# sailordiary/m3f.pytorch

Hardware: AMD Instinct MI355X
Metric: clips/sec (300-frame A+V, fwd+bwd) (higher is better)
Workload: dtype f32 (fp32-accurate products, fp32 accumulate: GEMMs as fp16x3 -- two fp16 terms per scaled operand, three MFMAs, error vs fp64 no larger than an fp32 GEMM's; the forward and backward recurrences at H=512 and H=256 as fp16x3 too (h is bounded; the backward producers split their values under a power-o

## Files before the change

### include/m3t_hip.h

```cpp
#ifndef M3T_HIP_H
#define M3T_HIP_H

#include <stddef.h>
#include <stdint.h>

#ifdef __cplusplus
extern "C" {
#endif

#define M3T_EINVAL 10001
#define M3T_MAX_SCANS 8
#define M3T_ESPIN 10002
#define M3T_SCAN_NO_PERSIST 1
#define M3T_SCAN_WHH 8
#define M3T_SCAN_FP32 4
#define M3T_SCAN_FAULT 16
#define M3T_SCAN_WIDE 32
#define M3T_BF16 2
#define M3T_GEMM_BACKGROUND 1
#define M3T_GEMM_BF16 2
#define M3T_GEMM_HIGH 256
#define M3T_GEMM_F16X3 1024
#define M3T_GEMM_BESIDE_SCAN 512
#define M3T_GEMM_EXCLUSIVE 8
// ... 59 lines not shown
typedef struct {
    const float* A; const float* B; float* C; const float* bias;
    const unsigned long long* amax_a; const unsigned long long* amax_b;
    int accumulate;
} m3t_window_problem;
int m3t_sgemm_window_batch(int n, const m3t_window_problem* problems, int transB, int n_seg, int win_len, int win_stride, int win_off,
                           int N, int K, int lda, int ldb, int ldc, int act, int flags, void* stream);

int m3t_absmax(int n, const float* const* x, const size_t* rows, const int* cols, const size_t* ld,
               unsigned long long* const* slots, void* stream);

int m3t_sgemm_plan(int transA, int M, int N, int K, int seg_len, size_t ws_bytes, int flags, int* kernel, int* splits);

int m3t_colsum(const float* X, int M, int N, int ld, float* out, int accumulate,
               float* ws, size_t ws_bytes, void* stream);

int m3t_transpose(const float* src, int R, int C, int lds, float* dst, int ldd, void* stream);

int m3t_relu_bwd(const float* a, float* dy, size_t n, void* stream);

typedef struct {
    const float* xproj;
    const float* w_hh;
    const float* b_hh;
    float* out;
    float* gates;
    float* h_n;
    int H, reverse, ldx, xoff, ldo, ooff;
} m3t_gru_fwd_desc;

// ... 267 lines not shown
```

### m3f.pytorch_amd/csrc/fuse_loss.hip

```cpp
#include "gru_common.h"
#include <cmath>
#include <cstdlib>
#include <mutex>

namespace {

__device__ __forceinline__ void fuse_weights(float sv, float sa, float& hv, float& ha, float& w0, float& w1) {
    hv = 1.f / (1.f + expf(-sv));
    ha = 1.f / (1.f + expf(-sa));
    const float m = fmaxf(hv, ha);
    const float ev = expf(hv - m), ea = expf(ha - m);
    const float inv = 1.f / (ev + ea);
    w0 = ev * inv;
    w1 = ea * inv;
}

__device__ __forceinline__ float mix2(float w0, float v, float w1, float a) { return fmaf(w0, v, w1 * a); }

__global__ __launch_bounds__(256) void att_fuse_fwd_kernel(const float* __restrict__ s_v, const float* __restrict__ s_a,
                                                           const float* __restrict__ x_v, const float* __restrict__ x_a,
                                                           float* __restrict__ f, int rows, int D, int vec) {
    const int lane = threadIdx.x & 63;
    const int row = blockIdx.x * 4 + (threadIdx.x >> 6);
    if (row >= rows) return;
    float hv, ha, w0, w1;
    fuse_weights(s_v[row], s_a[row], hv, ha, w0, w1);
    const size_t base = (size_t)row * D;
    if (vec) {
        const float4* pv = reinterpret_cast<const float4*>(x_v + base);
        const float4* pa = reinterpret_cast<const float4*>(x_a + base);
        float4* pf = reinterpret_cast<float4*>(f + base);
        for (int i = lane; i < (D >> 2); i += 64) {
            const float4 v = pv[i], a = pa[i];
            pf[i] = make_float4(mix2(w0, v.x, w1, a.x), mix2(w0, v.y, w1, a.y), mix2(w0, v.z, w1, a.z), mix2(w0, v.w, w1, a.w));
        }
    } else {
        for (int i = lane; i < D; i += 64) f[base + i] = mix2(w0, x_v[base + i], w1, x_a[base + i]);
    }
}

__global__ __launch_bounds__(256) void att_fuse_bwd_kernel(const float* __restrict__ df, const float* __restrict__ s_v,
                                                           const float* __restrict__ s_a, const float* __restrict__ x_v,
                                                           const float* __restrict__ x_a, float* __restrict__ ds_v,
                                                           float* __restrict__ ds_a, float* __restrict__ dx_v,
                                                           float* __restrict__ dx_a, int rows, int D, int vec) {
    const int lane = threadIdx.x & 63;
    const int row = blockIdx.x * 4 + (threadIdx.x >> 6);
    if (row >= rows) return;
    float hv, ha, w0, w1;
    fuse_weights(s_v[row], s_a[row], hv, ha, w0, w1);
    const size_t base = (size_t)row * D;
    float d0 = 0.f, d1 = 0.f;
    if (vec) {
// ... 445 lines not shown
}

extern "C" int m3t_sgd_step(float* p, const float* g, float* buf, size_t n, float lr, float momentum, float weight_decay,
                            int step, const float* guard, void* stream) {
    if (n == 0) return 0;
    if (!p || !g || !buf || step < 1) return M3T_EINVAL;
    int blocks = (int)((n + 255) / 256);
    if (blocks > 4096) blocks = 4096;
    sgd_kernel<<<blocks, 256, 0, (hipStream_t)stream>>>(p, g, buf, n, lr, momentum, weight_decay, step == 1, guard);
    M3T_LAUNCH_CHECK();
    return 0;
}

extern "C" int m3t_att_fuse_fwd(const float* s_v, const float* s_a, const float* x_v, const float* x_a, float* f,
                                int rows, int D, void* stream) {
    if (rows <= 0 || D <= 0) return 0;
    if (!s_v || !s_a || !x_v || !x_a || !f) return M3T_EINVAL;
    const int vec = (D % 4 == 0) && (((uintptr_t)x_v | (uintptr_t)x_a | (uintptr_t)f) % 16 == 0);
    att_fuse_fwd_kernel<<<cdiv(rows, 4), 256, 0, (hipStream_t)stream>>>(s_v, s_a, x_v, x_a, f, rows, D, vec);
    M3T_LAUNCH_CHECK();
    return 0;
}

extern "C" int m3t_att_fuse_bwd(const float* df, const float* s_v, const float* s_a, const float* x_v, const float* x_a,
                                float* ds_v, float* ds_a, float* dx_v, float* dx_a, int rows, int D, void* stream) {
    if (rows <= 0 || D <= 0) return 0;
    if (!df || !s_v || !s_a || !x_v || !x_a || !ds_v || !ds_a || !dx_v || !dx_a) return M3T_EINVAL;
    const int vec = (D % 4 == 0) &&
                    (((uintptr_t)x_v | (uintptr_t)x_a | (uintptr_t)df | (uintptr_t)dx_v | (uintptr_t)dx_a) % 16 == 0);
    att_fuse_bwd_kernel<<<cdiv(rows, 4), 256, 0, (hipStream_t)stream>>>(df, s_v, s_a, x_v, x_a, ds_v, ds_a, dx_v, dx_a,
                                                                         rows, D, vec);
    M3T_LAUNCH_CHECK();
    return 0;
}
// ... 86 lines not shown
```

### m3f.pytorch_amd/m3t/_lib.py

```python
import ctypes as C
import os

_HERE = os.path.dirname(os.path.abspath(__file__))
LIB_PATH = os.environ.get("M3T_LIB_PATH") or os.path.join(os.path.dirname(_HERE), "lib", "libm3t_hip.so")
CSRC_DIR = os.path.join(os.path.dirname(_HERE), "csrc")

M3T_EINVAL = 10001
M3T_ESPIN = 10002
M3T_SCAN_NO_PERSIST = 1
M3T_BF16 = 2
M3T_GEMM_BESIDE_SCAN = 512
M3T_GEMM_F16X3 = 1024
M3T_GEMM_HIGH = 256
M3T_GEMM_EXCLUSIVE = 8
M3T_CONV_IMAGES = 4096
M3T_SCAN_FP32 = 4
M3T_SCAN_WHH = 8
M3T_SCAN_FAULT = 16
M3T_SCAN_WIDE = 32
M3T_MAX_SCANS = 8

_f = C.c_void_p
_i = C.c_int
_z = C.c_size_t
# ... 37 lines not shown
    "m3t_conv3d_taps": [_f, _f, _f] + [_i] * 17 + [_f, _f, _f, _z, _f, _s],
    "m3t_sgemm_pre": [_i, _i, _i, _f, _i, _f, _i, _f, _i, _f, _i, _i, _f, _f, _s],
    "m3t_f16x3_split": [_f, _z, _i, _z, _f, _z, _f, _s],
    "m3t_f16x3_split_perm": [_f, _z, _i, _i, _z, _z, _z, _f, _f, _s],
    "m3t_f16x3_image_b": [_f, _i, _i, _z, _f, _f, _s],
    "m3t_sgemm_bimg": [_i, _i, _i, _f, _i, _f, _f, _i, _f, _i, _i, _f, _z, _f, _f, _s],
    "m3t_sgemm_ring": [_i, _i, _i, _i, _i, _f, _i, _f, _i, _f, _i, _f, _i, _i, _i, _i, _i, _i, _f, _z, _i, _f, _f, _i, _s],
    "m3t_conv3d_taps_pre": [_f, _f, _f] + [_i] * 16 + [_f, _f, _f, _z, _f, _s],
    "m3t_conv3d_fwd_taps": [_f, _f, _f, _f] + [_i] * 15 + [_f, _f, _f, _z, _f, _s],
    "m3t_conv3d_fwd_taps4": [_f, _f, _f, _f] + [_i] * 14 + [_f, _f, _f, _z, _f, _s],
    "m3t_planes_to_cl4": [_f, _f, _i, _i, C.c_longlong, _s],
    "m3t_conv3d_wgrad_taps": [_f, _f, _f] + [_i] * 16 + [_f, _f, _f, _z, _s],
    "m3t_amax_out": [C.c_void_p],
    "m3t_colsum": [_f, _i, _i, _i, _f, _i, _f, _z, _s],
    "m3t_transpose": [_f, _i, _i, _i, _f, _i, _s],
    "m3t_relu_bwd": [_f, _f, _z, _s],
    "m3t_gru_scan_fwd": [C.POINTER(GruFwdDesc), _i, _i, _i, _f, _z, _i, _s],
    "m3t_gru_scan_bwd": [C.POINTER(GruBwdDesc), _i, _i, _i, _f, _z, _i, _s],
    "m3t_gru_bwd_prepare_floats": [_i],
    "m3t_gru_bwd_prepare": [C.POINTER(C.c_void_p), _i, _i, _i, C.POINTER(C.c_void_p), _s],
    "m3t_gru_persist_count": [],
    "m3t_gru_scan_workgroups": [_i, _i, _i, _i, _i, _i],
    "m3t_gru_poll_error": [],
    "m3t_gru_error_reset": [],
    "m3t_gru_error_defer": [_i],
    "m3t_gru_inject_error": [_s],
    "m3t_gru_persist_owner": [],
    "m3t_gru_scan_arena": [C.c_void_p, _z],
    "m3t_gru_scan_arena_reset": [C.c_void_p],
    "m3t_gru_scan_after": [C.c_void_p],
# ... 142 lines not shown
```

### m3f.pytorch_amd/m3t/ops.py

```python
import ctypes as C
import os
import sys

import torch

from . import _lib
from ._lib import GruFwdDesc, GruBwdDesc, M3T_MAX_SCANS, M3THipError

_WS = {}
_WS_MIN = 64 << 20

PROFILE = []

import weakref

_GRAD_SINKS = {}


def register_grad_sink(param, view, owner=None):
    _GRAD_SINKS[id(param)] = [weakref.ref(param), view, False, id(owner) if owner is not None else None]


def clear_grad_sinks(owner=None):
    if owner is None:
# ... 431 lines not shown
        if drop is not None and drop[0] > 0:
            Cc = dy.shape[-1]
            _lib.check(lib().m3t_mask_pos_drop(_p(s), _p(dy), _p(out), dy.numel() // Cc, Cc, float(drop[0]), int(drop[1]), _stream()),
                       "m3t_mask_pos_drop")
            return out
        _lib.check(lib().m3t_mask_pos(_p(s), _p(dy), _p(mul), _p(out), dy.numel(), _stream()), "m3t_mask_pos")
        return out
    except BaseException:
        _amax_clear()
        raise


class _Linear(torch.autograd.Function):

    @staticmethod
    def forward(ctx, x, w, b, act, unit=False):
        x = _req(x.contiguous(), "x"); _req(w, "weight")
        K = x.shape[-1]
        N = w.shape[0]
        M = x.numel() // K
        y = torch.empty(x.shape[:-1] + (N,), dtype=x.dtype, device=x.device)
        ctx.prec = _PREC[0]
        slots = None
        ctx.w_slot = None
        if (ctx.prec & _lib.M3T_GEMM_F16X3) and M % 128 == 0 and N % 64 == 0 and K % 32 == 0 and w.is_contiguous():
            slots = amax_slots(3, x.device)
            ctx.w_keep = []
            ctx.w_slot = weight_amax(w, ctx.w_keep)
            ctx.x_slot = amax_one(x.device) if unit else slots.data_ptr()
            todo = ([] if unit else [(x, slots.data_ptr())]) + ([] if ctx.w_slot is not None else [(w, slots.data_ptr() + 8)])
            if todo and not measure_amax(todo):
                slots = None
            elif ctx.w_slot is None:
                ctx.w_slot = slots.data_ptr() + 8
        sgemm(0, 1, M, N, K, x, 0, K, w, 0, K, y, 0, N, bias=b, act=act, prec=ctx.prec, exclusive=True,
              amax=(None, None) if slots is None else (ctx.x_slot, ctx.w_slot))
        ctx.save_for_backward(x, w, y if act else None, slots)
        ctx.act, ctx.has_bias = act, b is not None
        ctx.bias_ref = b if (b is not None and id(b) in _GRAD_SINKS) else None
        ctx.weight_ref = w if id(w) in _GRAD_SINKS else None
        return y

    @staticmethod
    def backward(ctx, dy):
        x, w, y, slots = ctx.saved_tensors
        dy = _req(dy.contiguous(), "dy")
        if ctx.act:
            dy = mask_pos(y, dy)
        K, N = x.shape[-1], w.shape[0]
        M = x.numel() // K
        dx = dw = db = None
        a_x = a_w = a_dy = None
        if slots is not None and measure_amax([(dy, slots.data_ptr() + 16)]):
            a_x, a_w, a_dy = ctx.x_slot, ctx.w_slot, slots.data_ptr() + 16
        if ctx.needs_input_grad[0]:
            dx = torch.empty_like(x)
            sgemm(0, 0, M, K, N, dy, 0, N, w, 0, K, dx, 0, K, prec=ctx.prec, exclusive=True, amax=(a_dy, a_w))
        w_sink = _take_sink(ctx.weight_ref) if (ctx.needs_input_grad[1] and ctx.weight_ref is not None) else None
        b_sink = _take_sink(ctx.bias_ref) if (ctx.has_bias and ctx.needs_input_grad[2] and ctx.bias_ref is not None) else None
        if (ctx.needs_input_grad[1] and ctx.weight_ref is not None and w_sink is None) or \
                (ctx.has_bias and ctx.needs_input_grad[2] and ctx.bias_ref is not None and b_sink is None):
            join_wgrad(x.device)
        wg = wgrad_stream(x.device, _LINEAR_RR[0]) if x.is_cuda else None
        off_chain = on_stream(wg) if wg is not None else None
        if off_chain is not None and (w_sink is not None or b_sink is not None):
            wg.wait_stream(cur_stream())
        if ctx.needs_input_grad[1]:
            if w_sink is not None and off_chain is not None:
                with off_chain:
                    sgemm(1, 0, N, K, M, dy, 0, N, x, 0, K, w_sink, 0, K, prec=ctx.prec, amax=(a_dy, a_x))
                    if slots is not None:
                        slots.record_stream(wg)
            else:
                dw = w_sink if w_sink is not None else torch.empty_like(w)
                sgemm(1, 0, N, K, M, dy, 0, N, x, 0, K, dw, 0, K, prec=ctx.prec, exclusive=True, amax=(a_dy, a_x))
                if w_sink is not None:
                    dw = None
        if ctx.has_bias and ctx.needs_input_grad[2]:
            if b_sink is not None and off_chain is not None:
                with off_chain:
                    colsum(dy, 0, M, N, N, b_sink)
            else:
                db = b_sink if b_sink is not None else torch.empty(N, dtype=x.dtype, device=x.device)
                colsum(dy, 0, M, N, N, db)
                if b_sink is not None:
                    db = None
        if off_chain is not None and (w_sink is not None or b_sink is not None):
            dy.record_stream(wg)
            x.record_stream(wg)
            _WGRAD_PENDING[(x.device.type, x.device.index)] = True
            _LINEAR_RR[0] += 1
        return dx, dw, db, None, None


_LINEAR_RR = [0]


_NBT_PENDING = [None, 0]


def count_batch(counter):
    if counter is None:
        return
    if _NBT_PENDING[0] is not None:
        _NBT_PENDING[0].append(counter)
    else:
        counter.add_(1)


class batch_counters:
# ... 61 lines not shown
    @staticmethod
    def backward(ctx, dy):
        (y,) = ctx.saved_tensors
        return mask_pos(y, _req(dy.contiguous(), "dy"), drop=ctx.drop), None, None


def relu_dropout(y, p, seed=None):
    if p <= 0:
        return y
    if seed is None:
        seed = int(torch.empty(1, dtype=torch.int64).random_().item())
    return _ReluDropout.apply(y, float(p), int(seed))


def linear(x, w, b=None, act=0):
    return _Linear.apply(x, w, b, act, _is_unit(x))


SCAN_PER_STEP = [False]
SCAN_FAULT = [False]
RANGE_PROBE = [[] if os.environ.get("M3T_F16X3_PROBE") == "1" else None]


def _probe_range(tag, t2d):
    a = t2d.abs()
    rmax, cmax, gmax = a.amax(1), a.amax(0), a.max()
    big = torch.full((), float("inf"), device=t2d.device)
    lim = gmax * 2.0 ** -17
    sq = t2d.double() ** 2
    tot = sq.sum()
    past_r, past_c = rmax < lim, cmax < lim
# ... 291 lines not shown
        h_ns = [new(2 * L, B, Hs[s]) for s in range(n_stacks)]
        outs = [[new(B, T, 2 * Hs[s]) for s in range(n_stacks)] for _ in range(L)]
        cat_buf = None
        if cat_hi - cat_lo >= 2:
            cat_buf = new(B, T, sum(2 * Hs[s] for s in range(cat_lo, cat_hi)))
            off = 0
            for s in range(cat_lo, cat_hi):
                outs[L - 1][s] = cat_buf[..., off:off + 2 * Hs[s]]
                off += 2 * Hs[s]
        gates = [[new(2, B, T, 4 * Hs[s]) for s in range(n_stacks)] for _ in range(L)]
        xprojs = [[new(B, T, 6 * Hs[s]) for s in range(n_stacks)] for _ in range(L)]
        main = cur_stream()
        prec = _PREC[0]
        groups = _stream_groups(Hs, B)
        fslots = None
        if (prec & _lib.M3T_GEMM_F16X3) and all(h % 4 == 0 for h in Hs):
            fslots = amax_slots(n_stacks * (1 + 2 * L), dev)
            items = [(xs[s], fslots.data_ptr() + 8 * s) for s in range(n_stacks) if not (unit_mask >> s) & 1]
            wslot = {}
            ctx.w_keep = []
            for l in range(L):
                for s in range(n_stacks):
                    for d in (0, 1):
                        a = weight_amax(params[s][(2 * l + d) * 4], ctx.w_keep)
                        if a is None:
                            a = fslots.data_ptr() + 8 * (n_stacks + (l * n_stacks + s) * 2 + d)
                            items.append((params[s][(2 * l + d) * 4], a))
                        wslot[(l, s, d)] = a
            if not measure_amax(items):
                fslots = None
        one = amax_one(dev)

        def fslot_x(l, s):
            return None if fslots is None else (fslots.data_ptr() + 8 * s if (l == 0 and not (unit_mask >> s) & 1) else one)

        def fslot_w(l, s, d):
            return None if fslots is None else wslot[(l, s, d)]

        alone = not _interleaved(groups) and all(kind == "main" for kind, _ in groups)

        def level_fwd(l, idxs, scan, after=None, wide=False, progress=None):
            descs = []
            for s in idxs:
                H = Hs[s]
                inp = xs[s] if l == 0 else outs[l - 1][s]
                I = inp.shape[-1]
                for d in (0, 1):
                    w_ih, w_hh, b_ih, b_hh = params[s][(2 * l + d) * 4:(2 * l + d) * 4 + 4]
# ... 164 lines not shown
                    ctx.wfq_ev.record(wg1)
                ctx.wfq = wfq
        ctx.n_stacks, ctx.L, ctx.Hs, ctx.B, ctx.T, ctx.prec = n_stacks, L, Hs, B, T, prec
        ctx.unit_mask = unit_mask
        ctx.concurrent = concurrent
        ctx.cat = (cat_lo, cat_hi) if cat_buf is not None else (0, 0)
        saved = []
        for l in range(L):
            for s in range(n_stacks):
                saved += [outs[l][s], gates[l][s]]
        ctx.has_fslots = fslots is not None
        ctx.wslot = wslot if fslots is not None else None
        if fslots is not None:
            for st_ in (side_stream(dev),):
                fslots.record_stream(st_)
            saved.append(fslots)
        ctx.save_for_backward(*(list(tensors) + saved))
        result = []
        for s in range(n_stacks):
            if cat_buf is not None and cat_lo <= s < cat_hi:
                result += [cat_buf if s == cat_lo else new(0), h_ns[s]]
            else:
                result += [outs[L - 1][s], h_ns[s]]
        return tuple(result)

    @staticmethod
    def backward(ctx, *grads):
        n_stacks, L, Hs, B, T = ctx.n_stacks, ctx.L, ctx.Hs, ctx.B, ctx.T
        per = 1 + 8 * L
        st = ctx.saved_tensors
# ... 50 lines not shown
        main = cur_stream()
        groups = _stream_groups(Hs, B)
        cur = {s: douts[s] for s in range(n_stacks)}
        prec = ctx.prec
        wfq = ctx.wfq or {}
        if ctx.wfq_ev is not None:
            main.wait_event(ctx.wfq_ev)
        NSL = _CHUNK_WINDOWS + 1
        bslots = amax_slots(2 * L * n_stacks * NSL, dev) if fslots is not None else None
        one = amax_one(dev)

        def bslot(l, s, d, j=-1):
            return None if bslots is None else bslots.data_ptr() + 8 * (((l * n_stacks + s) * 2 + d) * NSL + 1 + j)

        def fslot_x(l, s):
            return None if fslots is None else (fslots.data_ptr() + 8 * s if (l == 0 and not (ctx.unit_mask >> s) & 1) else one)

        def fslot_w(l, s, d):
            return None if fslots is None else ctx.wslot[(l, s, d)]

        def chunk_plan(l, idxs):
            if bslots is None or len({Hs[i] for i in idxs}) != 1 or 2 * len(idxs) > M3T_MAX_SCANS or not any(need_dx[l][s] for s in idxs):
                return None
            H = Hs[idxs[0]]
            if H % 64 != 0 or any(need_dx[l][s] and layer_io(l, s)[0].shape[-1] % 64 != 0 for s in idxs) or not direct_whh:
                return None
            fl = _scan_flags(dev) | prec | _lib.M3T_SCAN_WHH | _lib.M3T_SCAN_WIDE
            if not lib().m3t_gru_scan_progress_ok(2 * len(idxs), H, B, T, fl, 1):
                return None
            tb = _chunk_bounds(B, T, backward=True)
# ... 221 lines not shown
                    for l in range(L - 1, -1, -1):
                        level_scan(l, idxs, progress=chunk_plan(l, idxs) if (kind == "main" and len(groups) == 1) else None)
                        level_gemms(l, idxs)
            for kind, _ in groups:
                if kind == "side":
                    main.wait_stream(side_stream(dev))
        for key_ in list(held):
            release_held(key_, None)
        weights_sunk = all(sunk[s * per + 1 + (2 * l + d) * 4 + j] for s in range(n_stacks) for l in range(L) for d in (0, 1) for j in (0, 1))
        if weights_sunk:
            for l in range(L):
                for s in range(n_stacks):
                    for t in (dgx[l][s], dgh[l][s]) + tuple(layer_io(l, s)[:2]):
                        for w_ in wgs:
                            t.record_stream(w_)
            for t in (bslots, fslots):
                if t is not None:
                    for w_ in wgs:
                        t.record_stream(w_)
            _WGRAD_PENDING[(dev.type, dev.index)] = True
        else:
            for w_ in wgs:
                main.wait_stream(w_)
        for s in range(n_stacks):
            out_grads[s * per] = dinp[0][s]
        return (None, None, None, None, None) + tuple(None if sunk[i] else g for i, g in enumerate(out_grads))


def multi_bigru(stacks, cat=None):
    L = stacks[0][2]
    flat = []
    for x, prm, l in stacks:
        if l != L:
            raise M3THipError("grouped GRU stacks must have the same depth")
        flat.append(x)
        flat.extend(prm)
    lo, hi = cat if cat is not None else (0, 0)
    unit_mask = sum(1 << i for i, (x, _, _) in enumerate(stacks) if _is_unit(x))
    res = _MultiBiGRU.apply(len(stacks), L, lo, hi, unit_mask, *flat)
    for i in range(len(stacks)):
        if res[2 * i].numel():
            res[2 * i]._m3t_unit = res[2 * i]._version + 1
    return [(res[2 * i], res[2 * i + 1]) for i in range(len(stacks))]


class _AttFuse(torch.autograd.Function):

    @staticmethod
    def forward(ctx, s_v, s_a, x_v, x_a):
        s_v, s_a = _req(s_v.contiguous(), "s_v"), _req(s_a.contiguous(), "s_a")
        x_v, x_a = _req(x_v.contiguous(), "x_v"), _req(x_a.contiguous(), "x_a")
        D = x_v.shape[-1]
        rows = x_v.numel() // D
        if x_a.shape != x_v.shape or s_v.numel() != rows or s_a.numel() != rows:
            raise M3THipError("att_fuse: shape mismatch")
        f = torch.empty_like(x_v)
        with _Timed("att_fuse_fwd_kernel", 1, 0, nbytes=4.0 * rows * (3 * D + 2)):
            _lib.check(lib().m3t_att_fuse_fwd(_p(s_v), _p(s_a), _p(x_v), _p(x_a), _p(f), rows, D, _stream()), "m3t_att_fuse_fwd")
        ctx.save_for_backward(s_v, s_a, x_v, x_a)
        return f

    @staticmethod
    def backward(ctx, df):
        s_v, s_a, x_v, x_a = ctx.saved_tensors
        df = _req(df.contiguous(), "df")
        D = x_v.shape[-1]
        rows = x_v.numel() // D
        ds_v, ds_a = torch.empty_like(s_v), torch.empty_like(s_a)
        dx_v, dx_a = torch.empty_like(x_v), torch.empty_like(x_a)
        with _Timed("att_fuse_bwd_kernel", 1, 0, nbytes=4.0 * rows * (5 * D + 4)):
            _lib.check(lib().m3t_att_fuse_bwd(_p(df), _p(s_v), _p(s_a), _p(x_v), _p(x_a), _p(ds_v), _p(ds_a), _p(dx_v),
                                              _p(dx_a), rows, D, _stream()), "m3t_att_fuse_bwd")
        return ds_v, ds_a, dx_v, dx_a


def att_fuse(s_v, s_a, x_v, x_a):
    return _AttFuse.apply(s_v, s_a, x_v, x_a)


class _VALoss(torch.autograd.Function):
    @staticmethod
    def forward(ctx, y_hat, valence, arousal, class_expr, expr_valid, iv, ia, n_expr, w_v, w_a, expr_w, use_mse):
        y = _req(y_hat.contiguous(), "y_hat")
        Cc = y.shape[-1]
        rows = y.numel() // Cc
        val = _req(valence.contiguous().float(), "valence")
        aro = _req(arousal.contiguous().float(), "arousal")
        cls = vld = None
        if n_expr > 0:
            cls = class_expr.contiguous().long()
            vld = expr_valid.contiguous().to(torch.uint8)
            if not cls.is_cuda or not vld.is_cuda:
# ... 356 lines not shown
        if wd is None:
            dx = _conv(da1, w1t, None, ds, None, None, B, T, Co, Ci, K, dil, 0, 1, prec, amax=(sl(7), sl(1)))
        else:
            dx = _conv(da1, w1t, None, None, None, None, B, T, Co, Ci, K, dil, 0, 1, prec, amax=(sl(7), sl(1)))
            sgemm(0, 0, B * T, Ci, Co, ds, 0, Co, wd, 0, Ci, dx, 0, Ci, accumulate=True, use_ws=False, prec=prec, amax=(sl(5), sl(3)))
            dwd = torch.empty_like(wd)
            sgemm(1, 0, Co, Ci, B * T, ds, 0, Co, x, 0, Ci, dwd, 0, Ci, prec=prec, amax=(sl(5), sl(0)))
            dbd = torch.empty(Co, dtype=torch.float32, device=dev)
            colsum(ds, 0, B * T, Co, Co, dbd)
        return dx, dv1, dg1, db1, dv2, dg2, db2, dwd, dbd, None, None, None, None, None, None


def temporal_block(x_btc, v1, g1, b1, v2, g2, b2, wd, bd, dilation, m1=None, m2=None, drop_p=0.0, seeds=(0, 0)):
    _LAST_OUT_SLOT[0] = None
    _X_EXT[0] = _tagged_amax(x_btc) if x_btc.is_contiguous() else None
    try:
        y = _TemporalBlock.apply(x_btc, v1, g1, b1, v2, g2, b2, wd, bd, dilation, m1, m2, float(drop_p), int(seeds[0]), int(seeds[1]))
    finally:
        _X_EXT[0] = None
    if _LAST_OUT_SLOT[0] is not None:
        y._m3t_amax = (_LAST_OUT_SLOT[0], y._version)
        _LAST_OUT_SLOT[0] = None
    return y


_LAST_OUT_SLOT = [None]
_X_EXT = [None]


class _ConvBnRelu(torch.autograd.Function):
# ... 1539 lines not shown
```

Baseline: 2831.

## Add thin-N linear kernels and fuse amax computation into att_fuse and GRU inputs

Adds dedicated HIP kernels for linear layers with few outputs (N<=16): the forward and dx kernels stage the weight in LDS, and dw uses a per-block partial-sum reduction with the bias gradient folded in. These replace general GEMM calls for heads and projections, and dx can apply a ReLU mask fused in. The attention-fusion forward now computes the output absmax in the same pass and tags it, so downstream fp16x3 GEMMs and GRU input scaling reuse that slot instead of running a separate absmax pass. This adds code paths, grid-stride loops with capped grids when amax is requested, and more slot-bookkeeping complexity.

```diff
diff --git a/include/m3t_hip.h b/include/m3t_hip.h
--- a/include/m3t_hip.h
+++ b/include/m3t_hip.h
@@ -97,6 +97,11 @@
 
 int m3t_colsum(const float* X, int M, int N, int ld, float* out, int accumulate,
                float* ws, size_t ws_bytes, void* stream);
+
+int m3t_linear_thin_fwd(const float* x, int ldx, const float* w, const float* bias, int act, float* y, int M, int K, int N, void* stream);
+int m3t_linear_thin_bwd_dx(const float* dy, const float* w, const float* relu_src, float* dx, int M, int K, int N, void* stream);
+int m3t_linear_thin_bwd_dw(const float* dy, const float* x, int ldx, float* dw, float* db, int M, int K, int N,
+                           float* ws, size_t ws_bytes, void* stream);
 
 int m3t_transpose(const float* src, int R, int C, int lds, float* dst, int ldd, void* stream);
 
diff --git a/m3f.pytorch_amd/csrc/fuse_loss.hip b/m3f.pytorch_amd/csrc/fuse_loss.hip
--- a/m3f.pytorch_amd/csrc/fuse_loss.hip
+++ b/m3f.pytorch_amd/csrc/fuse_loss.hip
@@ -19,24 +19,33 @@
 
 __global__ __launch_bounds__(256) void att_fuse_fwd_kernel(const float* __restrict__ s_v, const float* __restrict__ s_a,
                                                            const float* __restrict__ x_v, const float* __restrict__ x_a,
-                                                           float* __restrict__ f, int rows, int D, int vec) {
+                                                           float* __restrict__ f, int rows, int D, int vec, unsigned long long* amax) {
     const int lane = threadIdx.x & 63;
-    const int row = blockIdx.x * 4 + (threadIdx.x >> 6);
-    if (row >= rows) return;
-    float hv, ha, w0, w1;
-    fuse_weights(s_v[row], s_a[row], hv, ha, w0, w1);
-    const size_t base = (size_t)row * D;
-    if (vec) {
-        const float4* pv = reinterpret_cast<const float4*>(x_v + base);
-        const float4* pa = reinterpret_cast<const float4*>(x_a + base);
-        float4* pf = reinterpret_cast<float4*>(f + base);
-        for (int i = lane; i < (D >> 2); i += 64) {
-            const float4 v = pv[i], a = pa[i];
-            pf[i] = make_float4(mix2(w0, v.x, w1, a.x), mix2(w0, v.y, w1, a.y), mix2(w0, v.z, w1, a.z), mix2(w0, v.w, w1, a.w));
-        }
-    } else {
-        for (int i = lane; i < D; i += 64) f[base + i] = mix2(w0, x_v[base + i], w1, x_a[base + i]);
-    }
+    float mx = 0.f;
+    for (int row = blockIdx.x * 4 + (threadIdx.x >> 6); row < rows; row += gridDim.x * 4) {
+        float hv, ha, w0, w1;
+        fuse_weights(s_v[row], s_a[row], hv, ha, w0, w1);
+        const size_t base = (size_t)row * D;
+        if (vec) {
+            const float4* pv = reinterpret_cast<const float4*>(x_v + base);
+            const float4* pa = reinterpret_cast<const float4*>(x_a + base);
+            float4* pf = reinterpret_cast<float4*>(f + base);
+            for (int i = lane; i < (D >> 2); i += 64) {
+                const float4 v = pv[i], a = pa[i];
+                const float4 o = make_float4(mix2(w0, v.x, w1, a.x), mix2(w0, v.y, w1, a.y), mix2(w0, v.z, w1, a.z), mix2(w0, v.w, w1, a.w));
+                pf[i] = o;
+                mx = fmaxf(fmaxf(mx, m3t_fin_abs(o.x)), fmaxf(m3t_fin_abs(o.y), fmaxf(m3t_fin_abs(o.z), m3t_fin_abs(o.w))));
+            }
+        } else {
+            for (int i = lane; i < D; i += 64) {
+                const float o = mix2(w0, x_v[base + i], w1, x_a[base + i]);
+                f[base + i] = o;
+                mx = fmaxf(mx, m3t_fin_abs(o));
+            }
+        }
+    }
+    __shared__ float red4[4];
+    if (amax) m3t_block_raise_slot(amax, mx, red4);
 }
 
 __global__ __launch_bounds__(256) void att_fuse_bwd_kernel(const float* __restrict__ df, const float* __restrict__ s_v,
@@ -512,10 +521,13 @@
 
 extern "C" int m3t_att_fuse_fwd(const float* s_v, const float* s_a, const float* x_v, const float* x_a, float* f,
                                 int rows, int D, void* stream) {
+    unsigned long long* amax = m3t_take_amax_out();
     if (rows <= 0 || D <= 0) return 0;
     if (!s_v || !s_a || !x_v || !x_a || !f) return M3T_EINVAL;
     const int vec = (D % 4 == 0) && (((uintptr_t)x_v | (uintptr_t)x_a | (uintptr_t)f) % 16 == 0);
-    att_fuse_fwd_kernel<<<cdiv(rows, 4), 256, 0, (hipStream_t)stream>>>(s_v, s_a, x_v, x_a, f, rows, D, vec);
+    int grid = cdiv(rows, 4);
+    if (amax) grid = cdiv(grid, cdiv(grid, 512));
+    att_fuse_fwd_kernel<<<grid, 256, 0, (hipStream_t)stream>>>(s_v, s_a, x_v, x_a, f, rows, D, vec, amax);
     M3T_LAUNCH_CHECK();
     return 0;
 }
diff --git a/m3f.pytorch_amd/csrc/linear_thin.hip b/m3f.pytorch_amd/csrc/linear_thin.hip
--- /dev/null
+++ b/m3f.pytorch_amd/csrc/linear_thin.hip
@@ -0,0 +1,306 @@
+#include "common.h"
+
+namespace {
+
+constexpr int THIN_MAX_N = 16;
+constexpr int THIN_MAX_K = 2048;
+constexpr int THIN_F4 = 8;
+constexpr int THIN_DY_ROWS = 64;
+
+__device__ __forceinline__ float dot4(float acc, const float4& a, const float4& b) {
+#pragma clang fp contract(off)
+    acc = fmaf(a.x, b.x, acc);
+    acc = fmaf(a.y, b.y, acc);
+    acc = fmaf(a.z, b.z, acc);
+    acc = fmaf(a.w, b.w, acc);
+    return acc;
+}
+__device__ __forceinline__ void axpy4(float4& acc, float s, const float4& v) {
+#pragma clang fp contract(off)
+    acc.x = fmaf(s, v.x, acc.x);
+    acc.y = fmaf(s, v.y, acc.y);
+    acc.z = fmaf(s, v.z, acc.z);
+    acc.w = fmaf(s, v.w, acc.w);
+}
+
+__device__ __forceinline__ void stage_w(float4* s_w, const float* __restrict__ w, int n4) {
+    const float4* w4 = reinterpret_cast<const float4*>(w);
+    for (int i = threadIdx.x; i < n4; i += 256) s_w[i] = w4[i];
+    __syncthreads();
+}
+
+template <int G>
+__global__ __launch_bounds__(256) void linear_thin_fwd_kernel(const float* __restrict__ x, int ldx, const float* __restrict__ w,
+                                                              const float* __restrict__ bias, int act, float* __restrict__ y, int M, int K, int N) {
+#pragma clang fp contract(off)
+    extern __shared__ float4 s_w[];
+    const int K4 = K >> 2;
+    stage_w(s_w, w, N * K4);
+    constexpr int ROWS = 256 / G;
+    const int j = threadIdx.x % G, r = threadIdx.x / G;
+    for (long long row0 = (long long)blockIdx.x * ROWS; row0 < M; row0 += (long long)gridDim.x * ROWS) {
+        const long long m = row0 + r;
+        float acc[THIN_MAX_N];
+#pragma unroll
+        for (int n = 0; n < THIN_MAX_N; ++n) acc[n] = 0.f;
+        if (m < M) {
+            const float4* xr = reinterpret_cast<const float4*>(x + (size_t)m * ldx);
+            float4 xv[THIN_F4];
+#pragma unroll
+            for (int i = 0; i < THIN_F4; ++i) {
+                const int c = j + i * G;
+                xv[i] = c < K4 ? xr[c] : make_float4(0.f, 0.f, 0.f, 0.f);
+            }
+#pragma unroll
+            for (int i = 0; i < THIN_F4; ++i) {
+                const int c = j + i * G;
+                if (c < K4) {
+#pragma unroll
+                    for (int n = 0; n < THIN_MAX_N; ++n)
+                        if (n < N) acc[n] = dot4(acc[n], xv[i], s_w[n * K4 + c]);
+                }
+            }
+        }
+#pragma unroll
+        for (int n = 0; n < THIN_MAX_N; ++n)
+            if (n < N) {
+#pragma unroll
+                for (int o = G >> 1; o > 0; o >>= 1) acc[n] += __shfl_xor(acc[n], o, 64);
+            }
+        if (m < M) {
+#pragma unroll
+            for (int n = 0; n < THIN_MAX_N; ++n)
+                if (n < N && (n % G) == j) {
+                    float v = bias ? acc[n] + bias[n] : acc[n];
+                    if (act == 1) v = m3t_relu(v);
+                    y[(size_t)m * N + n] = v;
+                }
+        }
+    }
+}
+
+template <int G>
+__global__ __launch_bounds__(256) void linear_thin_dx_kernel(const float* __restrict__ dy, const float* __restrict__ w, const float* __restrict__ src,
+                                                             float* __restrict__ dx, int M, int K, int N, unsigned long long* amax) {
+#pragma clang fp contract(off)
+    extern __shared__ float4 s_w[];
+    const int K4 = K >> 2;
+    stage_w(s_w, w, N * K4);
+    constexpr int ROWS = 256 / G;
+    const int j = threadIdx.x % G, r = threadIdx.x / G;
+    float mx = 0.f;
+    for (long long row0 = (long long)blockIdx.x * ROWS; row0 < M; row0 += (long long)gridDim.x * ROWS) {
+        const long long m = row0 + r;
+        if (m < M) {
+            float d[THIN_MAX_N];
+#pragma unroll
+            for (int n = 0; n < THIN_MAX_N; ++n) d[n] = n < N ? dy[(size_t)m * N + n] : 0.f;
+            const float4* sr = src ? reinterpret_cast<const float4*>(src + (size_t)m * K) : nullptr;
+            float4* dr = reinterpret_cast<float4*>(dx + (size_t)m * K);
+#pragma unroll
+            for (int i = 0; i < THIN_F4; ++i) {
+                const int c = j + i * G;
+                if (c >= K4) break;
+                float4 a = make_float4(0.f, 0.f, 0.f, 0.f);
+#pragma unroll
+                for (int n = 0; n < THIN_MAX_N; ++n)
+                    if (n < N) axpy4(a, d[n], s_w[n * K4 + c]);
+                if (sr) {
+                    const float4 s = sr[c];
+                    a.x = s.x > 0.f ? a.x : 0.f; a.y = s.y > 0.f ? a.y : 0.f; a.z = s.z > 0.f ? a.z : 0.f; a.w = s.w > 0.f ? a.w : 0.f;
+                }
+                dr[c] = a;
+                mx = fmaxf(fmaxf(mx, m3t_fin_abs(a.x)), fmaxf(m3t_fin_abs(a.y), fmaxf(m3t_fin_abs(a.z), m3t_fin_abs(a.w))));
+            }
+        }
+    }
+    __shared__ float red4[4];
+    if (amax) m3t_block_raise_slot(amax, mx, red4);
+}
+
+constexpr int DW_THREADS = 512;
+__global__ __launch_bounds__(DW_THREADS) void linear_thin_dw_part_kernel(const float* __restrict__ dy, const float* __restrict__ x, int ldx,
+                                                                         float* __restrict__ part, int M, int K, int N, int rpb, int lg_tc) {
+#pragma clang fp contract(off)
+    __shared__ float s_dy[THIN_DY_ROWS * THIN_MAX_N];
+    __shared__ float4 s_red[DW_THREADS];
+    const int TC = 1 << lg_tc, RS = DW_THREADS >> lg_tc;
+    const int K4 = K >> 2, tc = threadIdx.x & (TC - 1), rs = threadIdx.x >> lg_tc;
+    const long long lo = (long long)blockIdx.x * rpb;
+    const int rows = (int)((lo + rpb <= M ? lo + rpb : (long long)M) - lo);
+    float* mine = part + (size_t)blockIdx.x * N * (K + 1);
+    for (int c0 = 0; c0 < K4; c0 += TC) {
+        const int c = c0 + tc;
+        float4 acc[THIN_MAX_N];
+        float dsum = 0.f;
+#pragma unroll
+        for (int n = 0; n < THIN_MAX_N; ++n) acc[n] = make_float4(0.f, 0.f, 0.f, 0.f);
+        for (int q0 = 0; q0 < rows; q0 += THIN_DY_ROWS) {
+            const int nq = rows - q0 < THIN_DY_ROWS ? rows - q0 : THIN_DY_ROWS;
+            __syncthreads();
+            for (int i = threadIdx.x; i < nq * N; i += DW_THREADS) s_dy[(i / N) * THIN_MAX_N + i % N] = dy[(size_t)(lo + q0) * N + i];
+            __syncthreads();
+            if (c0 == 0 && (int)threadIdx.x < N)
+                for (int q = 0; q < nq; ++q) dsum += s_dy[q * THIN_MAX_N + threadIdx.x];
+            if (c < K4) {
+                for (int qb = rs; qb < nq; qb += 8 * RS) {
+                    float4 xv[8];
+#pragma unroll
+                    for (int u = 0; u < 8; ++u) {
+                        const int q = qb + u * RS;
+                        xv[u] = q < nq ? reinterpret_cast<const float4*>(x + (size_t)(lo + q0 + q) * ldx)[c] : make_float4(0.f, 0.f, 0.f, 0.f);
+                    }
+#pragma unroll
+                    for (int u = 0; u < 8; ++u) {
+                        const int q = qb + u * RS;
+                        if (q < nq) {
+#pragma unroll
+                            for (int n = 0; n < THIN_MAX_N; ++n)
+                                if (n < N) axpy4(acc[n], s_dy[q * THIN_MAX_N + n], xv[u]);
+                        }
+                    }
+                }
+            }
+        }
+        if (c0 == 0 && (int)threadIdx.x < N) mine[(size_t)threadIdx.x * (K + 1) + K] = dsum;
+#pragma unroll
+        for (int n = 0; n < THIN_MAX_N; ++n)
+            if (n < N) {
+                float4 s = acc[n];
+                if (RS > 1) {
+                    __syncthreads();
+                    s_red[threadIdx.x] = s;
+                    __syncthreads();
+                    if (rs == 0)
+                        for (int k = 1; k < RS; ++k) {
+                            const float4 v = s_red[k * TC + tc];
+                            s.x += v.x; s.y += v.y; s.z += v.z; s.w += v.w;
+                        }
+                }
+                if (rs == 0 && c < K4) {
+                    float* o = mine + (size_t)n * (K + 1) + 4 * c;
+                    o[0] = s.x; o[1] = s.y; o[2] = s.z; o[3] = s.w;
+                }
+            }
+    }
+}
+
+__global__ __launch_bounds__(256) void linear_thin_dw_sum_kernel(const float* __restrict__ part, int P, float* __restrict__ dw, float* __restrict__ db,
+                                                                 int K, int N) {
+#pragma clang fp contract(off)
+    __shared__ float s_red[8][32];
+    const int total = N * (K + 1);
+    const int il = threadIdx.x & 31, sl = threadIdx.x >> 5;
+    const int i = blockIdx.x * 32 + il;
+    float s = 0.f;
+    if (i < total) {
+        for (int pb = sl; pb < P; pb += 64) {
+            float v[8];
+#pragma unroll
+            for (int u = 0; u < 8; ++u) {
+                const int p = pb + 8 * u;
+                v[u] = p < P ? part[(size_t)p * total + i] : 0.f;
+            }
+#pragma unroll
+            for (int u = 0; u < 8; ++u)
+                if (pb + 8 * u < P) s += v[u];
+        }
+    }
+    s_red[sl][il] = s;
+    __syncthreads();
+    if (sl == 0 && i < total) {
+#pragma unroll
+        for (int k = 1; k < 8; ++k) s += s_red[k][il];
+        const int n = i / (K + 1), k = i % (K + 1);
+        if (k < K) dw[(size_t)n * K + k] = s;
+        else if (db) db[n] = s;
+    }
+}
+
+int lanes_per_row(int K) {
+    const int K4 = K / 4;
+    int g = 1;
+    while (g < 64 && g * 8 < K4) g <<= 1;
+    return g;
+}
+
+bool aligned16(const void* p) { return ((uintptr_t)p & 15) == 0; }
+
+bool thin_shape_ok(int M, int K, int N) { return M >= 0 && N >= 1 && N <= THIN_MAX_N && K >= 4 && K % 4 == 0 && K <= THIN_MAX_K; }
+
+template <typename Kern>
+hipError_t allow_lds(Kern kern, size_t lds) {
+    return lds > 48 * 1024 ? hipFuncSetAttribute(reinterpret_cast<const void*>(kern), hipFuncAttributeMaxDynamicSharedMemorySize, (int)lds) : hipSuccess;
+}
+
+int row_grid(int M, int G, int cap) {
+    const int passes = cdiv(M, 256 / G);
+    return cdiv(passes, cdiv(passes, cap));
+}
+
+}
+
+#define THIN_BY_G(G_, ...)                       \
+    switch (G_) {                                \
+        case 1:  { constexpr int G = 1;  __VA_ARGS__; } break;  \
+        case 2:  { constexpr int G = 2;  __VA_ARGS__; } break;  \
+        case 4:  { constexpr int G = 4;  __VA_ARGS__; } break;  \
+        case 8:  { constexpr int G = 8;  __VA_ARGS__; } break;  \
+        case 16: { constexpr int G = 16; __VA_ARGS__; } break;  \
+        case 32: { constexpr int G = 32; __VA_ARGS__; } break;  \
+        default: { constexpr int G = 64; __VA_ARGS__; } break;  \
+    }
+
+extern "C" int m3t_linear_thin_fwd(const float* x, int ldx, const float* w, const float* bias, int act, float* y, int M, int K, int N,
+                                   void* stream) {
+    if (!thin_shape_ok(M, K, N) || !x || !w || !y || ldx < K || ldx % 4 != 0 || !aligned16(x) || !aligned16(w) || (act != 0 && act != 1))
+        return M3T_EINVAL;
+    if (M == 0) return 0;
+    const size_t lds = (size_t)N * K * sizeof(float);
+    const int g = lanes_per_row(K), grid = row_grid(M, g, 2048);
+    THIN_BY_G(g, {
+        hipError_t e = allow_lds(linear_thin_fwd_kernel<G>, lds);
+        if (e != hipSuccess) return (int)e;
+        linear_thin_fwd_kernel<G><<<grid, 256, lds, (hipStream_t)stream>>>(x, ldx, w, bias, act, y, M, K, N);
+    })
+    M3T_LAUNCH_CHECK();
+    return 0;
+}
+
+extern "C" int m3t_linear_thin_bwd_dx(const float* dy, const float* w, const float* relu_src, float* dx, int M, int K, int N, void* stream) {
+    unsigned long long* amax = m3t_take_amax_out();
+    if (!thin_shape_ok(M, K, N) || !dy || !w || !dx || !aligned16(w) || !aligned16(dx) || !aligned16(relu_src)) return M3T_EINVAL;
+    if (M == 0) return 0;
+    const size_t lds = (size_t)N * K * sizeof(float);
+    const int g = lanes_per_row(K), grid = row_grid(M, g, amax ? 512 : 2048);
+    THIN_BY_G(g, {
+        hipError_t e = allow_lds(linear_thin_dx_kernel<G>, lds);
+        if (e != hipSuccess) return (int)e;
+        linear_thin_dx_kernel<G><<<grid, 256, lds, (hipStream_t)stream>>>(dy, w, relu_src, dx, M, K, N, amax);
+    })
+    M3T_LAUNCH_CHECK();
+    return 0;
+}
+
+extern "C" int m3t_linear_thin_bwd_dw(const float* dy, const float* x, int ldx, float* dw, float* db, int M, int K, int N,
+                                      float* ws, size_t ws_bytes, void* stream) {
+    if (!thin_shape_ok(M, K, N) || !dy || !x || !dw || !ws || ldx < K || ldx % 4 != 0 || !aligned16(x) || ((uintptr_t)ws & 3) != 0)
+        return M3T_EINVAL;
+    const size_t per = (size_t)N * (K + 1) * sizeof(float);
+    if (ws_bytes < per) return M3T_EINVAL;
+    long long blocks = M / 32 > 1 ? M / 32 : 1;
+    if (blocks > 256) blocks = 256;
+    if ((size_t)blocks > ws_bytes / per) blocks = (long long)(ws_bytes / per);
+    const int rpb = M > 0 ? cdiv(M, (int)blocks) : 1;
+    const int P = M > 0 ? cdiv(M, rpb) : 0;
+    if (P > 0) {
+        const int K4 = K / 4;
+        int lg_tc = 0;
+        while (lg_tc < 9 && (1 << lg_tc) < K4) ++lg_tc;
+        linear_thin_dw_part_kernel<<<P, DW_THREADS, 0, (hipStream_t)stream>>>(dy, x, ldx, ws, M, K, N, rpb, lg_tc);
+        M3T_LAUNCH_CHECK();
+    }
+    linear_thin_dw_sum_kernel<<<cdiv(N * (K + 1), 32), 256, 0, (hipStream_t)stream>>>(ws, P, dw, db, K, N);
+    M3T_LAUNCH_CHECK();
+    return 0;
+}
diff --git a/m3f.pytorch_amd/m3t/_lib.py b/m3f.pytorch_amd/m3t/_lib.py
--- a/m3f.pytorch_amd/m3t/_lib.py
+++ b/m3f.pytorch_amd/m3t/_lib.py
@@ -75,6 +75,9 @@
     "m3t_amax_out": [C.c_void_p],
     "m3t_colsum": [_f, _i, _i, _i, _f, _i, _f, _z, _s],
     "m3t_transpose": [_f, _i, _i, _i, _f, _i, _s],
+    "m3t_linear_thin_fwd": [_f, _i, _f, _f, _i, _f, _i, _i, _i, _s],
+    "m3t_linear_thin_bwd_dx": [_f, _f, _f, _f, _i, _i, _i, _s],
+    "m3t_linear_thin_bwd_dw": [_f, _f, _i, _f, _f, _i, _i, _i, _f, _z, _s],
     "m3t_relu_bwd": [_f, _f, _z, _s],
     "m3t_gru_scan_fwd": [C.POINTER(GruFwdDesc), _i, _i, _i, _f, _z, _i, _s],
     "m3t_gru_scan_bwd": [C.POINTER(GruBwdDesc), _i, _i, _i, _f, _z, _i, _s],
diff --git a/m3f.pytorch_amd/m3t/ops.py b/m3f.pytorch_amd/m3t/ops.py
--- a/m3f.pytorch_amd/m3t/ops.py
+++ b/m3f.pytorch_amd/m3t/ops.py
@@ -469,13 +469,22 @@
 class _Linear(torch.autograd.Function):
 
     @staticmethod
-    def forward(ctx, x, w, b, act, unit=False):
+    def forward(ctx, x, w, b, act, unit=False, relu_in=False):
         x = _req(x.contiguous(), "x"); _req(w, "weight")
         K = x.shape[-1]
         N = w.shape[0]
         M = x.numel() // K
         y = torch.empty(x.shape[:-1] + (N,), dtype=x.dtype, device=x.device)
         ctx.prec = _PREC[0]
+        ctx.thin = _thin_ok(x, w, b, ctx.prec)
+        if ctx.thin:
+            _lib.check(lib().m3t_linear_thin_fwd(_p(x), K, _p(w), _p(b), int(act), _p(y), M, K, N, _stream()), "m3t_linear_thin_fwd")
+            ctx.relu_in = bool(relu_in)
+            ctx.save_for_backward(x, w, y if act else None, None)
+            ctx.act, ctx.has_bias = act, b is not None
+            ctx.bias_ref = b if (b is not None and id(b) in _GRAD_SINKS) else None
+            ctx.weight_ref = w if id(w) in _GRAD_SINKS else None
+            return y
         slots = None
         ctx.w_slot = None
         if (ctx.prec & _lib.M3T_GEMM_F16X3) and M % 128 == 0 and N % 64 == 0 and K % 32 == 0 and w.is_contiguous():
@@ -500,13 +509,21 @@
     def backward(ctx, dy):
         x, w, y, slots = ctx.saved_tensors
         dy = _req(dy.contiguous(), "dy")
+        g_slot = None
         if ctx.act:
-            dy = mask_pos(y, dy)
+            if _grad_masked(dy, y):
+                g_slot = _grad_slot(dy)[0]
+            else:
+                dy = mask_pos(y, dy)
         K, N = x.shape[-1], w.shape[0]
         M = x.numel() // K
+        if ctx.thin:
+            return _thin_backward(ctx, x, w, dy, M, K, N)
         dx = dw = db = None
         a_x = a_w = a_dy = None
-        if slots is not None and measure_amax([(dy, slots.data_ptr() + 16)]):
+        if slots is not None and g_slot is not None:
+            a_x, a_w, a_dy = ctx.x_slot, ctx.w_slot, g_slot.data_ptr()
+        elif slots is not None and measure_amax([(dy, slots.data_ptr() + 16)]):
             a_x, a_w, a_dy = ctx.x_slot, ctx.w_slot, slots.data_ptr() + 16
         if ctx.needs_input_grad[0]:
             dx = torch.empty_like(x)
@@ -526,6 +543,8 @@
                     sgemm(1, 0, N, K, M, dy, 0, N, x, 0, K, w_sink, 0, K, prec=ctx.prec, amax=(a_dy, a_x))
                     if slots is not None:
                         slots.record_stream(wg)
+                    if g_slot is not None:
+                        g_slot.record_stream(wg)
             else:
                 dw = w_sink if w_sink is not None else torch.empty_like(w)
                 sgemm(1, 0, N, K, M, dy, 0, N, x, 0, K, dw, 0, K, prec=ctx.prec, exclusive=True, amax=(a_dy, a_x))
@@ -545,10 +564,85 @@
             x.record_stream(wg)
             _WGRAD_PENDING[(x.device.type, x.device.index)] = True
             _LINEAR_RR[0] += 1
-        return dx, dw, db, None, None
+        return dx, dw, db, None, None, None
 
 
 _LINEAR_RR = [0]
+
+LINEAR_THIN = [os.environ.get("M3T_LINEAR_THIN", "1") != "0"]
+
+
+def _thin_ok(x, w, b, prec):
+    if not LINEAR_THIN[0] or (prec & _lib.M3T_BF16) or w.dim() != 2 or not w.is_contiguous() or w.dtype != torch.float32:
+        return False
+    N, K = w.shape
+    return (1 <= N <= 16 and K % 4 == 0 and 4 <= K <= 2048 and x.shape[-1] == K and x.numel() // K < 2 ** 31 and x.data_ptr() % 16 == 0
+            and w.data_ptr() % 16 == 0 and (b is None or (b.dtype == torch.float32 and b.is_contiguous() and b.numel() == N)))
+
+
+_GRAD_MASKED = {}
+
+
+def _note_grad_masked(t, src):
+    if len(_GRAD_MASKED) > 64:
+        _GRAD_MASKED.clear()
+    _GRAD_MASKED[id(t)] = (weakref.ref(t), t._version, t.data_ptr(), src.data_ptr(), src.numel())
+
+
+def _grad_masked(t, y):
+    e = _GRAD_MASKED.pop(id(t), None)
+    return (e is not None and e[0]() is t and e[1] == t._version and e[2] == t.data_ptr() and y is not None and e[3] == y.data_ptr()
+            and e[4] == y.numel() == t.numel())
+
+
+def _thin_backward(ctx, x, w, dy, M, K, N):
+    dx = dw = db = None
+    if ctx.needs_input_grad[0]:
+        dx = torch.empty_like(x)
+        slot = amax_slots(1, x.device) if ctx.relu_in else None
+        amax_out(slot.data_ptr() if slot is not None else None)
+        try:
+            _lib.check(lib().m3t_linear_thin_bwd_dx(_p(dy), _p(w), _p(x) if ctx.relu_in else None, _p(dx), M, K, N, _stream()),
+                       "m3t_linear_thin_bwd_dx")
+        except BaseException:
+            _amax_clear()
+            raise
+        if slot is not None:
+            _note_grad_slot(dx, slot)
+            _note_grad_masked(dx, x)
+    need_w = ctx.needs_input_grad[1]
+    need_b = ctx.has_bias and ctx.needs_input_grad[2]
+    w_sink = _take_sink(ctx.weight_ref) if (need_w and ctx.weight_ref is not None) else None
+    b_sink = _take_sink(ctx.bias_ref) if (need_b and ctx.bias_ref is not None) else None
+    if (need_w and ctx.weight_ref is not None and w_sink is None) or (need_b and ctx.bias_ref is not None and b_sink is None):
+        join_wgrad(x.device)
+    if not need_w:
+        if need_b:
+            db = b_sink if b_sink is not None else torch.empty(N, dtype=x.dtype, device=x.device)
+            colsum(dy, 0, M, N, N, db)
+            if b_sink is not None:
+                db = None
+        return dx, None, db, None, None, None
+    wg = wgrad_stream(x.device, _LINEAR_RR[0]) if x.is_cuda else None
+    off = wg is not None and w_sink is not None and (b_sink is not None or not need_b)
+    dw = w_sink if w_sink is not None else torch.empty_like(w)
+    db = (b_sink if b_sink is not None else torch.empty(N, dtype=x.dtype, device=x.device)) if need_b else None
+
+    def run():
+        ws = workspace(x.device)
+        _lib.check(lib().m3t_linear_thin_bwd_dw(_p(dy), _p(x), K, _p(dw), _p(db), M, K, N, _p(ws), ws.numel() * 4, _stream()),
+                   "m3t_linear_thin_bwd_dw")
+    if off:
+        wg.wait_stream(cur_stream())
+        with on_stream(wg):
+            run()
+        dy.record_stream(wg)
+        x.record_stream(wg)
+        _WGRAD_PENDING[(x.device.type, x.device.index)] = True
+        _LINEAR_RR[0] += 1
+    else:
+        run()
+    return dx, (None if w_sink is not None else dw), (None if (b_sink is not None or not need_b) else db), None, None, None
 
 
 _NBT_PENDING = [None, 0]
@@ -640,7 +734,11 @@
 
 
 def linear(x, w, b=None, act=0):
-    return _Linear.apply(x, w, b, act, _is_unit(x))
+    relu_in = isinstance(x, torch.Tensor) and getattr(x, "_m3t_relu", None) == x._version and x.is_contiguous()
+    y = _Linear.apply(x, w, b, act, _is_unit(x), relu_in)
+    if act == 1:
+        y._m3t_relu = y._version
+    return y
 
 
 SCAN_PER_STEP = [False]
@@ -962,9 +1060,10 @@
         prec = _PREC[0]
         groups = _stream_groups(Hs, B)
         fslots = None
+        x_ext = ctx.x_ext = dict(_GRU_X_SLOT[0])
         if (prec & _lib.M3T_GEMM_F16X3) and all(h % 4 == 0 for h in Hs):
             fslots = amax_slots(n_stacks * (1 + 2 * L), dev)
-            items = [(xs[s], fslots.data_ptr() + 8 * s) for s in range(n_stacks) if not (unit_mask >> s) & 1]
+            items = [(xs[s], fslots.data_ptr() + 8 * s) for s in range(n_stacks) if not (unit_mask >> s) & 1 and s not in x_ext]
             wslot = {}
             ctx.w_keep = []
             for l in range(L):
@@ -980,6 +1079,8 @@
         one = amax_one(dev)
 
         def fslot_x(l, s):
+            if fslots is not None and l == 0 and s in x_ext:
+                return x_ext[s].data_ptr()
             return None if fslots is None else (fslots.data_ptr() + 8 * s if (l == 0 and not (unit_mask >> s) & 1) else one)
 
         def fslot_w(l, s, d):
@@ -1174,6 +1275,8 @@
         if fslots is not None:
             for st_ in (side_stream(dev),):
                 fslots.record_stream(st_)
+                for t_ in x_ext.values():
+                    t_.record_stream(st_)
             saved.append(fslots)
         ctx.save_for_backward(*(list(tensors) + saved))
         result = []
@@ -1254,6 +1357,8 @@
             return None if bslots is None else bslots.data_ptr() + 8 * (((l * n_stacks + s) * 2 + d) * NSL + 1 + j)
 
         def fslot_x(l, s):
+            if fslots is not None and l == 0 and s in ctx.x_ext:
+                return ctx.x_ext[s].data_ptr()
             return None if fslots is None else (fslots.data_ptr() + 8 * s if (l == 0 and not (ctx.unit_mask >> s) & 1) else one)
 
         def fslot_w(l, s, d):
@@ -1505,7 +1610,7 @@
                     for t in (dgx[l][s], dgh[l][s]) + tuple(layer_io(l, s)[:2]):
                         for w_ in wgs:
                             t.record_stream(w_)
-            for t in (bslots, fslots):
+            for t in (bslots, fslots) + (tuple(ctx.x_ext.values()) if fslots is not None else ()):
                 if t is not None:
                     for w_ in wgs:
                         t.record_stream(w_)
@@ -1528,11 +1633,19 @@
         flat.extend(prm)
     lo, hi = cat if cat is not None else (0, 0)
     unit_mask = sum(1 << i for i, (x, _, _) in enumerate(stacks) if _is_unit(x))
-    res = _MultiBiGRU.apply(len(stacks), L, lo, hi, unit_mask, *flat)
+    _GRU_X_SLOT[0] = {i: t for i, t in ((i, _tagged_amax(x) if x.is_contiguous() else None) for i, (x, _, _) in enumerate(stacks))
+                      if torch.is_tensor(t) and t.numel() == 1 and not (unit_mask >> i) & 1}
+    try:
+        res = _MultiBiGRU.apply(len(stacks), L, lo, hi, unit_mask, *flat)
+    finally:
+        _GRU_X_SLOT[0] = {}
     for i in range(len(stacks)):
         if res[2 * i].numel():
             res[2 * i]._m3t_unit = res[2 * i]._version + 1
     return [(res[2 * i], res[2 * i + 1]) for i in range(len(stacks))]
+
+
+_GRU_X_SLOT = [{}]
 
 
 class _AttFuse(torch.autograd.Function):
@@ -1546,8 +1659,15 @@
         if x_a.shape != x_v.shape or s_v.numel() != rows or s_a.numel() != rows:
             raise M3THipError("att_fuse: shape mismatch")
         f = torch.empty_like(x_v)
+        slot = amax_slots(1, f.device)
         with _Timed("att_fuse_fwd_kernel", 1, 0, nbytes=4.0 * rows * (3 * D + 2)):
-            _lib.check(lib().m3t_att_fuse_fwd(_p(s_v), _p(s_a), _p(x_v), _p(x_a), _p(f), rows, D, _stream()), "m3t_att_fuse_fwd")
+            amax_out(slot.data_ptr())
+            try:
+                _lib.check(lib().m3t_att_fuse_fwd(_p(s_v), _p(s_a), _p(x_v), _p(x_a), _p(f), rows, D, _stream()), "m3t_att_fuse_fwd")
+            except BaseException:
+                _amax_clear()
+                raise
+        _OUT_SLOT[0] = slot
         ctx.save_for_backward(s_v, s_a, x_v, x_a)
         return f
 
@@ -1566,7 +1686,8 @@
 
 
 def att_fuse(s_v, s_a, x_v, x_a):
-    return _AttFuse.apply(s_v, s_a, x_v, x_a)
+    _OUT_SLOT[0] = None
+    return _tag_out(_AttFuse.apply(s_v, s_a, x_v, x_a))
 
 
 class _VALoss(torch.autograd.Function):
@@ -1953,6 +2074,8 @@
 def temporal_block(x_btc, v1, g1, b1, v2, g2, b2, wd, bd, dilation, m1=None, m2=None, drop_p=0.0, seeds=(0, 0)):
     _LAST_OUT_SLOT[0] = None
     _X_EXT[0] = _tagged_amax(x_btc) if x_btc.is_contiguous() else None
+    if not isinstance(_X_EXT[0], tuple):
+        _X_EXT[0] = None
     try:
         y = _TemporalBlock.apply(x_btc, v1, g1, b1, v2, g2, b2, wd, bd, dilation, m1, m2, float(drop_p), int(seeds[0]), int(seeds[1]))
     finally:
```

Result: faster. 2862 (median of 6 runs) (+1.1%).
